# kabkabm/defensegan

Hardware: NVIDIA H100
Metric: reconstructed images/sec at R=10,L=200 (higher is better)
Workload: dtype f16

## Files before the change

### defensegan_b200/csrc/dgan_api.cu

```cuda
#include <algorithm>
#include <cmath>
#include <cstdio>
#include <cstring>
#include <memory>
#include <new>

#include "common.cuh"
#include "kernels_simt.cuh"
#include "kernels_tc.cuh"
#include "kernels_tc2.cuh"
#include "kernels_vjp.cuh"

namespace dgan {

static thread_local std::string g_last_error;
void set_error(const std::string& msg) { g_last_error = msg; }

PairTable deconv_fwd_pairs(int h_in, int w_in, int h_used, int w_used, int in_raster) {
  if (in_raster <= 0) in_raster = w_in;
  PairTable t;
  t.off.push_back(0);
  for (int i = 0; i < h_used; ++i)
    for (int j = 0; j < w_used; ++j) {
      for (int ka = 0; ka < 5; ++ka) {
// ... 1311 lines not shown
  return h->kind_names[kind].c_str();
}

int dgan_profile_read(dgan_handle h, int max_kinds, double* ms_out, int64_t* launches_out, double* flops_per_launch_out) {
  if (h == nullptr || ms_out == nullptr || launches_out == nullptr || flops_per_launch_out == nullptr) return DGAN_ERR_INVALID_ARG;
  const int nk = std::min(max_kinds, (int)h->kind_names.size());
  for (int k = 0; k < nk; ++k) {
    ms_out[k] = 0.0; launches_out[k] = 0;
    flops_per_launch_out[k] = 2.0 * h->kind_macs_per_row[k] * (double)h->n_rows_cur;
  }
  for (auto& r : h->prof) {
    DGAN_CUDA_CHECK(cudaEventSynchronize(r.b));
    float ms = 0.f;
    DGAN_CUDA_CHECK(cudaEventElapsedTime(&ms, r.a, r.b));
    if (r.kind >= 0 && r.kind < nk) { ms_out[r.kind] += ms; launches_out[r.kind]++; }
    cudaEventDestroy(r.a); cudaEventDestroy(r.b);
  }
  h->prof.clear();
  return DGAN_OK;
}

static int check_plans_impl(const dgan_desc* d, int n_rows, int n_pairs, int mutate, TcPass pass) {
  using namespace dgan;
  if (d == nullptr || n_rows <= 0 || n_pairs <= 0) { set_error("invalid argument"); return DGAN_ERR_INVALID_ARG; }
  const int n_pad = ((n_rows + 2 * kRowTile - 1) / (2 * kRowTile)) * 2 * kRowTile, n_mpairs = n_pad / (2 * kRowTile);
  Widths wd;
  if (int rc = padded_widths(d, &wd)) return rc;
  const std::string wide_target = pass == TC_PASS_TANGENT ? "Generator.3.jvp" : pass == TC_PASS_WEIGHTED ? "last.fwd.w" : "Generator.3.fwd";
  for (const TcDir& dr : tc_directions(d, pass)) {
    if (int rc = tc_dir_supported(dr)) return rc;
    Tc2Plan plan;
    int rc = tc2_plan(dr.N, dr.K, dr.tab, dr.h_grid, dr.w_grid, dr.max_acc, 0, dr.epi, dr.out_bytes, n_mpairs, n_pairs, &plan);
    if (rc) { set_error(dr.name + ": " + dgan_last_error()); return rc; }
    const bool narrow = mutate >= 12 && dr.name == "last.bwd", wide = mutate != 0 && mutate < 12 && dr.name == wide_target;
    if ((narrow || wide) && plan.stream_m.size() > 40) {
      auto mma = [&](size_t i, auto f) { TcMmaRec m = TcMmaRec::decode(plan.stream_m[i]); f(m); plan.stream_m[i] = m.encode(); };
      auto producer = [&](size_t i, auto f) { TcProducerRec p = TcProducerRec::decode(plan.stream_p[i]); f(p); plan.stream_p[i] = p.encode(); };
      auto every_mma = [&](auto f) { for (size_t i = 0; i < plan.stream_m.size(); ++i) mma(i, f); };
      switch (mutate) {
        case 1: mma(20, [](TcMmaRec& m) {
                  TcOp op = TcOp::decode(m.ops[0]);
                  op.first ^= 1u;
                  m.ops[0] = op.encode();
                });
                break;
        case 2: mma(20, [](TcMmaRec& m) {
                  for (uint32_t j = 1; j < m.maxb; ++j)
                    if (m.ops[j] != m.ops[0]) { std::swap(m.ops[0], m.ops[j]); break; }
                });
                break;
        case 3: producer(20, [](TcProducerRec& p) { p.tile[0] ^= 1u; }); break;
        case 4: producer(20, [](TcProducerRec& p) { p.pix[0] ^= 1u; }); break;
        case 5: producer(20, [](TcProducerRec& p) { p.kc ^= 1u; }); break;
        case 6: plan.eitems[0] = -1; break;
        case 7: for (size_t i = 0; i < plan.stream_p.size(); ++i)
                  producer(i, [](TcProducerRec& p) { p.dep = TC2_NSLOT; });
                break;
        case 8: producer(20, [](TcProducerRec& p) { p.off = 0xBF; }); break;
        case 9: std::swap(plan.stream_m[20], plan.stream_m[21]);
                std::swap(plan.stream_p[20], plan.stream_p[21]);
                break;
        case 10: plan.maxb = 3;
                 every_mma([](TcMmaRec& m) { m.maxb = 3; });
                 break;
        case 11: every_mma([](TcMmaRec& m) { m.maxb = 2; }); break;
        case 12: every_mma([&](TcMmaRec& m) { m.ksub = plan.ksub == 1 ? 2 : 1; }); break;
        case 13: producer(20, [](TcProducerRec& p) { p.kc |= 1u; }); break;
        default: break;
      }
    }
    std::string err;
    if ((rc = tc2_check_plan(dr.N, dr.K, dr.tab, n_mpairs, dr.epi, dr.out_bytes, plan, &err))) { set_error(dr.name + ": " + err); return rc; }
    if (mutate != 0) continue;
    for (const Tc2Kind& k : kTc2Kinds) {
      if (k.n != dr.N || k.ksub != plan.ksub || k.epi != dr.epi || k.out_bytes != dr.out_bytes || k.maxb == plan.maxb) continue;
      Tc2Plan forced;
      if ((rc = tc2_plan(dr.N, dr.K, dr.tab, dr.h_grid, dr.w_grid, dr.max_acc, k.maxb, dr.epi, dr.out_bytes, n_mpairs, n_pairs, &forced))) {
        set_error(dr.name + " (" + std::to_string(k.maxb) + " slots): " + dgan_last_error());
        return rc;
      }
      if ((rc = tc2_check_plan(dr.N, dr.K, dr.tab, n_mpairs, dr.epi, dr.out_bytes, forced, &err))) {
        set_error(dr.name + " (" + std::to_string(k.maxb) + " slots): " + err);
        return rc;
      }
    }
  }
  return 0;
}

int dgan_debug_check_plans(const dgan_desc* d, int n_rows, int n_pairs, int mutate) {
  return check_plans_impl(d, n_rows, n_pairs, mutate, TC_PASS_PROJ);
}

int dgan_debug_check_tangent_plans(const dgan_desc* d, int n_rows, int n_pairs, int mutate) {
  return check_plans_impl(d, n_rows, n_pairs, mutate, TC_PASS_TANGENT);
}

int dgan_debug_check_weighted_plans(const dgan_desc* d, int n_rows, int n_pairs, int mutate) {
  return check_plans_impl(d, n_rows, n_pairs, mutate, TC_PASS_WEIGHTED);
}
// ... 62 lines not shown
    const bool forced = (int)di == force_dir;
    const int rc = tc2_plan(dr.N, dr.K, dr.tab, dr.h_grid, dr.w_grid, dr.max_acc, forced ? force_maxb : 0, dr.epi, dr.out_bytes,
                            n_mpairs, n_pairs, &plan, forced ? force_shape : nullptr);
    if (rc) return -1;
    char line[320];
    const double mb = (double)plan.n_bytes / 1e6;
    total += mb;
    snprintf(line, sizeof line, "%s | %d | %d | %dx%d, %dx%d | %zu | %d | %lld | %lld | %.1f | %.3f | %.1f | %d | %.1f | %.1f | %lld | %s/f%d\n",
             dr.name.c_str(), dr.N, dr.K, plan.shape[0], plan.shape[1], plan.shape[2], plan.shape[3],
             plan.hdrs.size() * (size_t)n_mpairs, plan.n_slots, plan.n_steps, plan.n_mma, mb, plan.load_max / std::max(plan.load_mean, 1.0),
             100.0 * (double)plan.n_pad / (double)std::max(plan.n_mma, 1LL), plan.maxb, plan.op_ns_max / 1e3,
             plan.load_max / 1e3, plan.n_mma * plan.ksub, epi_name(dr.epi), 8 * dr.out_bytes);
    out += line;
  }
  char line[64];
  snprintf(line, sizeof line, "total staged MB per L-step | %.1f\n", total);
  out += line;
  const int n = (int)std::min(out.size(), (size_t)buf_len - 1);
  memcpy(buf, out.data(), (size_t)n);
  buf[n] = 0;
  return n;
}

int dgan_debug_plan_stats_slots(const dgan_desc* d, int n_rows, int n_pairs, int force_dir, int force_maxb, char* buf, int buf_len) {
  return plan_stats_impl(d, n_rows, n_pairs, force_dir, force_maxb, nullptr, buf, buf_len);
}

int dgan_debug_plan_stats_window(const dgan_desc* d, int n_rows, int n_pairs, int force_dir, int force_maxb, int wh, int ww,
                                 int sy, int sx, char* buf, int buf_len) {
  const int shape[4] = {wh, ww, sy, sx};
  return plan_stats_impl(d, n_rows, n_pairs, force_dir, force_maxb, shape, buf, buf_len);
}

int dgan_debug_padded_widths(const dgan_desc* d, int* out) {
  using namespace dgan;
  if (d == nullptr || out == nullptr) { set_error("invalid argument"); return DGAN_ERR_INVALID_ARG; }
  Widths w;
  if (int rc = padded_widths(d, &w)) return rc;
  out[0] = w.latent; out[1] = w.c4; out[2] = w.c2; out[3] = w.c1;
  return 0;
}

static int workspace_layout_impl(dgan_handle h, int n_rows, char* buf, int buf_len, bool weighted) {
  if (h == nullptr || n_rows <= 0 || buf == nullptr || buf_len <= 0) { set_error("invalid argument"); return -1; }
  std::string out;
  carve(h, n_rows, nullptr, &out, weighted);
  if (out.size() + 1 > (size_t)buf_len) { set_error("buffer too small"); return -1; }
  memcpy(buf, out.c_str(), out.size() + 1);
  return (int)out.size();
}

int dgan_debug_workspace_layout(dgan_handle h, int n_rows, char* buf, int buf_len) {
  return workspace_layout_impl(h, n_rows, buf, buf_len, false);
}

int dgan_debug_workspace_layout_weighted(dgan_handle h, int n_rows, char* buf, int buf_len) {
  return workspace_layout_impl(h, n_rows, buf, buf_len, true);
}

int dgan_debug_plan_stats(const dgan_desc* d, int n_rows, int n_pairs, char* buf, int buf_len) {
  return dgan_debug_plan_stats_slots(d, n_rows, n_pairs, -1, 0, buf, buf_len);
}

}
```

### defensegan_b200/csrc/kernels_tc2.cuh

```cuda
#pragma once
#include "kernels_tc.cuh"
#include "tc_records.cuh"

namespace dgan {

constexpr int TC2_SMEM_MAX = 232448;
constexpr int TC2_TILE_BYTES = 128 * 128;
constexpr int TC2_BUF_COLS = 256;
constexpr int TC2_CONSUMERS = 256;
constexpr int TC2_THREADS = TC2_CONSUMERS + 128;
constexpr int TC2_PRODUCER_REGS = 40, TC2_CONSUMER_REGS = 232;
constexpr int TC2_STORE_ROWS = 16;

constexpr int TC2_MAX_PAIRS = 80;
struct Tc2Heads {
  uint32_t off[TC2_MAX_PAIRS + 1];
};

struct __align__(16) TcItem2 {
  uint16_t q[16];
  uint32_t n_acc;
};
static_assert(sizeof(TcItem2) == 48 && offsetof(TcItem2, n_acc) == 32, "the kernel's item loads");

__host__ __device__ constexpr int tc2_acc_stride(int n_tile) { return n_tile <= 32 ? 32 : (n_tile < 64 ? 64 : n_tile); }

__host__ __device__ constexpr bool tc2_tma_epilogue(int n_tile, int epi, int out_bytes) {
  return out_bytes == 2 && n_tile >= 64 && epi != EPI_FINAL_SIGMOID1 && epi != EPI_FINAL_TANH3 && epi != EPI_FINAL_SIGMOID1_W &&
         epi != EPI_FINAL_TANH3_W;
}

constexpr int TC2_REC_BATCH = 16;
constexpr int TC2_STAGING_BYTES = TC2_REC_BATCH * (int)sizeof(TcRec);
constexpr int TC2_MREC_BYTES = TC2_NSLOT * (int)sizeof(TcRec);

__host__ __device__ constexpr int tc2_epi_tiles(int n_tile, int epi, int out_bytes) {
  return tc2_tma_epilogue(n_tile, epi, out_bytes) ? 2 : 0;
}
__host__ __device__ constexpr int tc2_ksub(int K) { return K % 64 == 0 ? 4 : K / 16; }
__host__ __device__ constexpr int tc2_a_bytes(int ksub) { return 128 * 32 * ksub; }
__host__ __device__ constexpr int tc2_b_bytes(int n_tile, int ksub) { return n_tile * 32 * ksub; }
__host__ __device__ constexpr int tc2_zero_bytes(int n_tile, int maxb, int ksub) { return maxb > 1 ? tc2_b_bytes(n_tile, ksub) : 0; }
__host__ __device__ constexpr int tc2_ring_bytes(int n_tile, int maxb, int ksub, int epi, int out_bytes) {
  const int epi_b = tc2_epi_tiles(n_tile, epi, out_bytes) * TC2_TILE_BYTES;
  const int raw = ((TC2_SMEM_MAX - 1024 - 256 - TC2_MREC_BYTES - TC2_STAGING_BYTES - epi_b - tc2_zero_bytes(n_tile, maxb, ksub)) / 1024) * 1024;
  return raw > TC2_RING_MAX_KB * 1024 ? TC2_RING_MAX_KB * 1024 : raw;
}

template <int N_TILE, int MAXB_, int KSUB_ = 4, int EPI = EPI_NONE, int OUT_BYTES = 2>
struct Tc2Cfg {
  static_assert(MAXB_ >= 1 && MAXB_ <= TC2_BUF_COLS / tc2_acc_stride(N_TILE), "more accumulator slots than columns");
  static_assert(KSUB_ >= 1 && KSUB_ <= 4, "k16 MMAs per op");
  static constexpr int KSUB = KSUB_;
  static constexpr int A_BYTES = tc2_a_bytes(KSUB);
  static constexpr int B_TILE = tc2_b_bytes(N_TILE, KSUB);
  static constexpr int A_SUB = 128 * 32, B_SUB = N_TILE * 32;
  static constexpr int MAXB = MAXB_;
  static constexpr int ACC_REGS = MAXB * N_TILE / 2;
  static constexpr bool TMA_EPI = tc2_tma_epilogue(N_TILE, EPI, OUT_BYTES);
  static constexpr int EPI_TILES = tc2_epi_tiles(N_TILE, EPI, OUT_BYTES);
  static constexpr int EPI_BYTES = EPI_TILES * TC2_TILE_BYTES;
  static constexpr int ZERO_BYTES = tc2_zero_bytes(N_TILE, MAXB, KSUB);
  static constexpr int RING_BYTES = tc2_ring_bytes(N_TILE, MAXB, KSUB, EPI, OUT_BYTES);
  static constexpr int SMEM_BYTES = RING_BYTES + ZERO_BYTES + EPI_BYTES + TC2_STAGING_BYTES + 1024 + 256 + TC2_MREC_BYTES;
};

#define TC2_KINDS(X)                                                                                                   \
  X(256, 1, 4, EPI_BIAS_RELU, __half) X(256, 1, 4, EPI_BIAS, __half) X(256, 1, 4, EPI_MASK, __half)                    \
  X(256, 1, 4, EPI_NONE, __half) X(256, 1, 4, EPI_NONE, float) X(256, 1, 4, EPI_BIAS, float)                           \
  X(128, 2, 4, EPI_BIAS_RELU, __half) X(128, 2, 4, EPI_BIAS, __half) X(128, 2, 4, EPI_MASK, __half)                    \
  X(128, 2, 4, EPI_NONE, __half) X(128, 2, 4, EPI_NONE, float) X(128, 2, 4, EPI_BIAS, float)                           \
  X(128, 1, 4, EPI_NONE, float)                                                                                        \
  X(64, 4, 4, EPI_BIAS_RELU, __half) X(64, 4, 4, EPI_BIAS, __half) X(64, 4, 4, EPI_MASK, __half)                      \
  X(64, 4, 4, EPI_NONE, __half) X(64, 4, 4, EPI_NONE, float) X(64, 4, 4, EPI_BIAS, float)                              \
// ... 62 lines not shown
__device__ __forceinline__ uint2 ld_shared_v2(uint32_t addr) {
  uint2 v;
  asm volatile("ld.shared.v2.b32 {%0, %1}, [%2];" : "=r"(v.x), "=r"(v.y) : "r"(addr));
  return v;
}
__device__ __forceinline__ uint4 ld_shared_v4(uint32_t addr) {
  uint4 v;
  asm volatile("ld.shared.v4.b32 {%0, %1, %2, %3}, [%4];" : "=r"(v.x), "=r"(v.y), "=r"(v.z), "=r"(v.w) : "r"(addr));
  return v;
}
__device__ __forceinline__ uint4 ld_shared_v4_ordered(uint32_t addr) {
  uint4 v;
  asm volatile("ld.shared.v4.b32 {%0, %1, %2, %3}, [%4];" : "=r"(v.x), "=r"(v.y), "=r"(v.z), "=r"(v.w) : "r"(addr) : "memory");
  return v;
}
__device__ __forceinline__ void bulk_load(uint32_t dst, const void* src, uint32_t bytes, uint32_t bar) {
  asm volatile("cp.async.bulk.shared::cluster.global.mbarrier::complete_tx::bytes [%0], [%1], %2, [%3];"
               ::"r"(dst), "l"(src), "r"(bytes), "r"(bar) : "memory");
}
__device__ __forceinline__ void wgmma_wait1() { asm volatile("wgmma.wait_group.sync.aligned 1;" ::: "memory"); }
template <int R> __device__ __forceinline__ void setmaxnreg_inc() { asm volatile("setmaxnreg.inc.sync.aligned.u32 %0;" ::"n"(R)); }
template <int R> __device__ __forceinline__ void setmaxnreg_dec() { asm volatile("setmaxnreg.dec.sync.aligned.u32 %0;" ::"n"(R)); }
__device__ __forceinline__ bool elect_one() {
  uint32_t pred;
  asm volatile("{\n\t.reg .pred P1;\n\telect.sync _|P1, 0xffffffff;\n\tselp.u32 %0, 1, 0, P1;\n\t}" : "=r"(pred));
  return pred != 0;
}
}

__device__ __forceinline__ int tc2_item_at(const int* __restrict__ order, int k, int pair, int n_pairs, int n_slots) {
  return k < n_slots ? __ldg(order + (size_t)k * n_pairs + pair) : -1;
}

template <int NT, int MAXB, int KSUB, int NREG>
__device__ __forceinline__ void tc2_mma_round(float (&acc)[NREG], const uint32_t (&q)[6], uint64_t da0, uint64_t db0, uint32_t zoff) {
  constexpr uint32_t DA_K = KSUB == 4 ? 2u : (uint32_t)(128 * 32 >> 4), DB_K = KSUB == 4 ? 2u : (uint32_t)(NT * 32 >> 4);
#pragma unroll
  for (int a = 0; a < MAXB; ++a) {
    const uint32_t e = TcMmaRec::Ops::get(q[a / TcMmaRec::Ops::PER_WORD], a);
    const uint32_t bs = TcOp::Slot::get(e);
    const uint64_t da = da0 + (uint64_t)(TcOp::A::get(e) * (uint32_t)(tc2_a_bytes(KSUB) >> 4));
    const uint64_t db = db0 + (uint64_t)(bs == (uint32_t)TC2_ZERO_SLOT ? zoff : bs * (uint32_t)(tc2_b_bytes(NT, KSUB) >> 4));
    const uint32_t keep = TcOp::First::get(e) ^ 1u;
#pragma unroll
    for (int k = 0; k < KSUB; ++k) ptx::Wgmma<NT>::mma(acc + a * (NT / 2), da + DA_K * k, db + DB_K * k, k > 0 ? 1u : keep);
  }
}

template <int MAXB>
__device__ __forceinline__ void tc2_pop_round(uint32_t (&q)[6]) {
  using Ops = TcMmaRec::Ops;
  static_assert(Ops::WORDS == 6, "the op queue holds every op word");
  if constexpr (MAXB >= Ops::PER_WORD) {
#pragma unroll
    for (int i = 0; i < 6; ++i) q[i] = (i + MAXB / Ops::PER_WORD < 6) ? q[i + MAXB / Ops::PER_WORD] : 0u;
  } else {
#pragma unroll
    for (int i = 0; i < 5; ++i) q[i] = __funnelshift_r(q[i], q[i + 1], Ops::BITS * MAXB);
    q[5] >>= Ops::BITS * MAXB;
  }
}

#ifdef DGAN_PROBE
constexpr int TC2_PROBE_WORDS = 16;
__device__ unsigned long long g_tc2_probe[48][160][TC2_PROBE_WORDS];
__device__ __forceinline__ unsigned long long probe_gtime() {
  unsigned long long t;
  asm volatile("mov.u64 %0, %%globaltimer;" : "=l"(t));
  return t;
}
__device__ __forceinline__ long long probe_clock_after(uint32_t w0) {
  long long t;
  asm volatile("{\n\t.reg .pred p;\n\tsetp.ge.s32 p, %1, 0;\n\tmov.u64 %0, 0;\n\t@p mov.u64 %0, %%clock64;\n\t}" : "=l"(t) : "r"(w0) : "memory");
  return t;
}
__host__ __device__ constexpr int tc2_probe_key(int n_tile, int epi, int out_bytes) {
  return (n_tile == 256 ? 0 : n_tile == 128 ? 1 : n_tile == 64 ? 2 : n_tile == 48 ? 3 : 4) * 8 + (out_bytes == 4 ? 6 : (epi < 4 ? epi : epi - 4));
}
// ... 18 lines not shown
  extern __shared__ uint8_t smem_raw[];
#ifdef DGAN_PROBE
  const long long probe_t_start = clock64();
  const unsigned long long probe_g_start = probe_gtime();
  long long probe_wait_full = 0, probe_issue = 0, probe_wait1 = 0, probe_wait0 = 0, probe_epi = 0;
  unsigned probe_rec = 0, probe_head = 0, probe_steps = 0;
#endif
  const uint32_t smem_base = (ptx::smem_u32(smem_raw) + 1023u) & ~1023u;
  const uint32_t zero_base = smem_base + Cfg::RING_BYTES;
  const uint32_t epi_base = zero_base + Cfg::ZERO_BYTES;
  const uint32_t stg_base = epi_base + Cfg::EPI_BYTES;
  const uint32_t bar_base = stg_base + TC2_STAGING_BYTES;
  const uint32_t bar_full = bar_base, bar_empty = bar_base + 64, mrec_base = bar_base + 256;

  const int warp = threadIdx.x >> 5, lane = threadIdx.x & 31;
  const uint32_t rank = ptx::cluster_ctarank();
  const int pair = blockIdx.x >> 1, n_pairs = gridDim.x >> 1;
  const uint32_t rbeg = heads.off[pair], rend = heads.off[pair + 1];

  uint4 mine = make_uint4(0, 0, 0, 0);
  if (warp == PRODUCER) {
    if (2 * rbeg + lane < 2 * rend) mine = __ldg(reinterpret_cast<const uint4*>(stream_p + rbeg) + lane);
    if (lane == 0) {
      ptx::prefetch_tmap(&tm_a);
      ptx::prefetch_tmap(&tm_b);
      if (TMA_EPI) ptx::prefetch_tmap(&tm_out);
      for (int s = 0; s < TC2_NSLOT; ++s) {
        ptx::mbar_init(bar_full + 8 * s, 1);
        ptx::mbar_init(bar_empty + 8 * s, 2 * TC2_CONSUMERS / 32);
      }
      ptx::fence_barrier_init();
    }
  }
  if constexpr (Cfg::ZERO_BYTES > 0) {
    if (threadIdx.x < TC2_CONSUMERS) {
      for (uint32_t i = threadIdx.x; i < (uint32_t)Cfg::ZERO_BYTES / 16u; i += TC2_CONSUMERS) ptx::st_shared_v4(zero_base + 16u * i, 0u, 0u, 0u, 0u);
      ptx::fence_proxy_async_smem();
    }
  }
  ptx::cluster_sync();
#ifdef DGAN_PROBE
  const long long probe_t_entry = clock64();
#endif
  pdl_launch_dependents();
  pdl_wait();
#ifdef DGAN_PROBE
  const long long probe_t_go = clock64();
  unsigned probe_h0 = (unsigned)probe_t_go;
  bool probe_new_item = true;
#endif

  if (warp >= PRODUCER) {
    ptx::setmaxnreg_dec<TC2_PRODUCER_REGS>();
    if (warp == PRODUCER) {
      const TcRec* __restrict__ stream = stream_p;
      uint32_t it = 0;
      const uint32_t ring = stg_base;
      for (uint32_t base = rbeg; base < rend; base += TC2_REC_BATCH) {
        ptx::st_shared_v4(ring + lane * 16u, mine.x, mine.y, mine.z, mine.w);
        __syncwarp();
        if (2 * (base + TC2_REC_BATCH) + lane < 2 * rend) mine = __ldg(reinterpret_cast<const uint4*>(stream + base + TC2_REC_BATCH) + lane);
        const uint32_t cnt = min((uint32_t)TC2_REC_BATCH, rend - base);
        for (uint32_t i = 0; i < cnt; ++i, ++it) {
          const uint4 r0 = ptx::ld_shared_v4(ring + i * 32u);
          const uint2 r1 = ptx::ld_shared_v2(ring + i * 32u + 16u);
          const uint32_t slot = it & (TC2_NSLOT - 1);
          using P = TcProducerRec;
// ... 60 lines not shown
#ifdef DGAN_PROBE
        const long long probe_w0 = clock64();
        if (probe_new_item) probe_head += (unsigned)probe_w0 - probe_h0;
        probe_new_item = false;
#endif
        ptx::mbar_wait(bar_full + 8 * slot, phase);
#ifdef DGAN_PROBE
        const long long probe_w1 = clock64();
        probe_wait_full += probe_w1 - probe_w0;
        if (it == 0 && threadIdx.x == 0) g_tc2_probe[tc2_probe_key(N_TILE, EPI, (int)sizeof(TOUT))][blockIdx.x][7] = probe_gtime();
#endif
        const uint4 r0 = ptx::ld_shared_v4_ordered(mrec_base + slot * (uint32_t)sizeof(TcRec));
        const uint4 r1 = ptx::ld_shared_v4_ordered(mrec_base + slot * (uint32_t)sizeof(TcRec) + 16u);
        flags = TcMmaRec::Flags::get(r0.x);
#ifdef DGAN_PROBE
        const unsigned probe_rec_step = (unsigned)probe_clock_after(r0.x) - (unsigned)probe_w1;
        probe_rec += probe_rec_step;
#endif
        const int nA = TcMmaRec::NA::get(r0.x), n_rounds = TcMmaRec::Rounds::get(r0.x);
        const uint32_t sa = smem_base + (TcMmaRec::Off::get(r0.x) << 10);
        const uint64_t da0 = KSUB == 4 ? make_smem_desc_sw128(sa + (uint32_t)wg * 64u * 128u) : make_smem_desc_sw32(sa + (uint32_t)wg * 64u * 32u);
        const uint32_t sb = sa + (uint32_t)nA * A_BYTES;
        const uint64_t db0 = KSUB == 4 ? make_smem_desc_sw128(sb) : make_smem_desc_sw32(sb);
        const uint32_t zoff = (zero_base - sb) >> 4;
        uint32_t q[6] = {r0.z, r0.w, r1.x, r1.y, r1.z, r1.w};
#ifdef DGAN_PROBE
        long long probe_step_wait = 0;
#endif
        ptx::fence_operands(acc);
        ptx::wgmma_fence();
        for (int r = 0; r < n_rounds; ++r) {
          tc2_mma_round<N_TILE, Cfg::MAXB, KSUB>(acc, q, da0, db0, zoff);
          tc2_pop_round<Cfg::MAXB>(q);
          ptx::wgmma_commit();
#ifdef DGAN_PROBE
          const long long probe_c0 = clock64();
#endif
          ptx::wgmma_wait1();
#ifdef DGAN_PROBE
          probe_step_wait += clock64() - probe_c0;
#endif
          if (r == 0) {
            __syncwarp();
            if (!(flags & TcMmaRec::FIRST) && lane < 2) ptx::mbar_arrive_cluster(bar_empty + 8 * ((it - 1) & (TC2_NSLOT - 1)), (uint32_t)lane);
          }
        }
        ptx::fence_operands(acc);
#ifdef DGAN_PROBE
        probe_wait1 += probe_step_wait;
        probe_issue += clock64() - probe_w1 - probe_step_wait - probe_rec_step;
#endif
        ++ri; ++it;
      } while (!(flags & TcMmaRec::LAST));
#ifdef DGAN_PROBE
      const long long probe_d0 = clock64();
#endif
      ptx::wgmma_wait0();
      ptx::fence_operands(acc);
#ifdef DGAN_PROBE
      const long long probe_e0 = clock64();
      probe_wait0 += probe_e0 - probe_d0;
#endif
      __syncwarp();
      if (lane < 2) ptx::mbar_arrive_cluster(bar_empty + 8 * ((it - 1) & (TC2_NSLOT - 1)), (uint32_t)lane);

      const int mp = tc2_item_mp(item_e);
      auto q_of = [&](int a) { return (int)__shfl_sync(0xffffffffu, q_mine, a); };
// ... 237 lines not shown
};
static uint32_t tc2_box_k(int K) { return tc2_ksub(K) == 4 ? 64u : 16u; }
struct TcDir {
  std::string name, kind;
  int N = 0, K = 0, P_in = 0, P_out = 0, n_tiles = 0;
  PairTable tab;
  int h_grid = 0, w_grid = 0;
  int max_acc = 1;
  int epi = EPI_NONE, out_bytes = 2, bias_pstride = 0;
  int ld = 0, col0 = 0, out_ld = 0;
  int n_real = 0;
  std::string base_kind;
  __half* w = nullptr;
  CUtensorMap tm_b{};
  int force_maxb = 0;
  std::vector<std::pair<int, Tc2Schedule>> by_mpairs;
};

static int tc2_maxb(int N) { return TC2_BUF_COLS / tc2_acc_stride(N); }

struct Tc2HostStep {
  int kc = 0, nA = 0, nB = 0, n_rounds = 0;
  int a_pix[TC2_MAX_A] = {0, 0, 0, 0};
  uint8_t b_ent[TC2_MAX_BSLOTS] = {0};
  uint8_t ops[TC2_OP_BYTES] = {0};
  int n_real = 0;
  int bytes = 0;
};
struct Tc2HostItem {
  TcItem2 hdr{};
  std::vector<Tc2HostStep> steps;
  double stage_bytes = 0.0;
  long long n_ops = 0;
};

static void tc2_build_item(const PairTable& tab, const std::vector<int>& qs, int N, int K, int max_b, int max_a,
                           int step_max_bytes, Tc2HostItem* out) {
  const int ksub = tc2_ksub(K), kch = K / (16 * ksub), a_bytes = tc2_a_bytes(ksub), b_tile = tc2_b_bytes(N, ksub);
  out->hdr = TcItem2{};
  out->hdr.n_acc = (uint32_t)qs.size();
  for (size_t a = 0; a < qs.size(); ++a) out->hdr.q[a] = (uint16_t)qs[a];
  out->steps.clear();
  std::vector<std::pair<int, std::vector<std::pair<int, int>>>> by_p;
  for (size_t a = 0; a < qs.size(); ++a)
    for (int e = tab.off[qs[a]]; e < tab.off[qs[a] + 1]; ++e) {
      const int p = tab.pairs[e].x, t = tab.pairs[e].y;
      size_t g = 0;
      for (; g < by_p.size(); ++g)
        if (by_p[g].first == p) break;
      if (g == by_p.size()) by_p.push_back({p, {}});
      by_p[g].second.push_back({t, (int)a});
    }
  std::sort(by_p.begin(), by_p.end(), [](const auto& l, const auto& r) { return l.first < r.first; });
  for (auto& g : by_p)
    std::stable_sort(g.second.begin(), g.second.end(), [](const auto& l, const auto& r) { return l.second < r.second; });
  std::vector<std::pair<int, std::vector<std::pair<int, int>>>> px;
  const int ent_cap = std::min(TC2_MAX_BSLOTS, std::max(1, (step_max_bytes - a_bytes) / b_tile));
  for (auto& g : by_p)
    for (size_t b0 = 0; b0 < g.second.size(); b0 += (size_t)ent_cap)
      px.push_back({g.first, std::vector<std::pair<int, int>>(g.second.begin() + b0,
                                                               g.second.begin() + std::min(g.second.size(), b0 + (size_t)ent_cap))});
  const int max_rounds = TC2_OP_BYTES / max_b;
  struct Group { size_t i0, i1; };
  std::vector<Group> groups;
  {
    size_t i0 = 0;
// ... 35 lines not shown
    st.nA = (int)(G.i1 - G.i0);
    std::fill(st.ops, st.ops + TC2_OP_BYTES, TC2_PAD_OP);
    int slot_of[32], cnt[8] = {0, 0, 0, 0, 0, 0, 0, 0};
    for (int t = 0; t < 32; ++t) slot_of[t] = -1;
    for (size_t i = G.i0; i < G.i1; ++i) {
      st.a_pix[i - G.i0] = px[i].first;
      for (auto& ta : px[i].second) {
        const int t = ta.first, acc = ta.second;
        if (slot_of[t] < 0) {
          slot_of[t] = st.nB;
          st.b_ent[st.nB++] = (uint8_t)t;
        }
        const bool first = !(seen & (1u << acc));
        const int r = cnt[acc]++;
        st.ops[r * max_b + acc] = TcOp{(uint32_t)(i - G.i0), (uint32_t)slot_of[t], first ? 1u : 0u}.encode();
        st.n_rounds = std::max(st.n_rounds, r + 1);
        st.n_real += 1;
        seen |= 1u << acc;
      }
    }
    st.bytes = st.nA * a_bytes + st.nB * b_tile;
    out->steps.push_back(st);
  }
  const size_t n_groups = out->steps.size();
  for (int kc = 1; kc < kch; ++kc)
    for (size_t gi = 0; gi < n_groups; ++gi) {
      Tc2HostStep sk = out->steps[gi];
      sk.kc = kc;
      for (int o = 0; o < TC2_OP_BYTES; ++o) sk.ops[o] = (uint8_t)TcOp::First::put(sk.ops[o], 0u);
      out->steps.push_back(sk);
    }
  out->stage_bytes = 0.0;
  out->n_ops = 0;
  for (auto& stp : out->steps) { out->stage_bytes += stp.bytes; out->n_ops += (long long)stp.n_rounds * max_b; }
}

static void tc2_enumerate_windows(int h_grid, int w_grid, int wh, int ww, int sy, int sx, std::vector<std::vector<int>>* wins) {
  wins->clear();
  for (int by = 0; by < h_grid; by += wh * sy)
    for (int bx = 0; bx < w_grid; bx += ww * sx)
      for (int ry = 0; ry < sy; ++ry)
        for (int rx = 0; rx < sx; ++rx) {
          std::vector<int> qs;
          for (int i = 0; i < wh; ++i)
            for (int j = 0; j < ww; ++j) {
              const int y = by + ry + i * sy, x = bx + rx + j * sx;
              if (y < h_grid && x < w_grid) qs.push_back(y * w_grid + x);
            }
          if (!qs.empty()) wins->push_back(qs);
        }
}

#ifndef DGAN_STEP_MAX_KB
#define DGAN_STEP_MAX_KB 48
#endif
#ifndef DGAN_STEP_MAX_KB_N64
#define DGAN_STEP_MAX_KB_N64 64
#endif
#ifndef DGAN_COST_EPI_KB
#define DGAN_COST_EPI_KB 24.0
#endif
#ifndef DGAN_COST_FIXED_KB
#define DGAN_COST_FIXED_KB 48.0
#endif
#ifndef DGAN_COST_NS_PER_KB
#define DGAN_COST_NS_PER_KB 6.8
#endif
#ifndef DGAN_COST_OP_NS
#define DGAN_COST_OP_NS 103.0
#endif
#ifndef DGAN_COST_STEP_NS
#define DGAN_COST_STEP_NS 942.0
#endif
#ifndef DGAN_COST_OP_MIN_N
#define DGAN_COST_OP_MIN_N 32
#endif
#ifndef TC2_REFINE_BUDGET
#define TC2_REFINE_BUDGET (1LL << 26)
#endif

struct Tc2Plan {
  int shape[4] = {1, 1, 1, 1};
  int n_slots = 0, n_pairs = 0;
  std::vector<TcItem2> hdrs;
  std::vector<TcRec> stream_p, stream_m;
  std::vector<uint32_t> stream_off;
  std::vector<int> eitems;
  long long n_mma = 0, n_pad = 0, n_steps = 0, n_bytes = 0;
  double load_max = 0.0, load_mean = 0.0;
  double op_ns_max = 0.0;
  int maxb = 1, ring_bytes = 0;
  int ksub = 4;
};

static double tc2_op_ns(int N, int ksub) {
  return DGAN_COST_OP_NS * (double)std::max(N, DGAN_COST_OP_MIN_N) / 64.0 * (double)ksub / 4.0;
}

static int tc2_search(int N, int K, const PairTable& tab, int h_grid, int w_grid, int max_acc, int force_maxb, int epi,
                      int out_bytes, int n_mpairs, int n_pairs, const int* force_shape, Tc2Plan* plan,
                      std::vector<Tc2HostItem>* best_items, std::vector<std::vector<int>>* best_lists) {
  const int max_a = TC2_MAX_A;
  const int step_kb = (N == 64 && K == 128) ? DGAN_STEP_MAX_KB_N64 : DGAN_STEP_MAX_KB;
  const int ksub = tc2_ksub(K);
  const double op_ns = tc2_op_ns(N, ksub);
  double best_cost = 1e300;
  plan->maxb = 0;
  std::vector<std::vector<int>> wins;
  for (const Tc2Kind& kind : kTc2Kinds) {
    if (kind.n != N || kind.ksub != ksub || kind.epi != epi || kind.out_bytes != out_bytes) continue;
    if (force_maxb > 0 && kind.maxb != force_maxb) continue;
    const int mb = kind.maxb, ring = tc2_ring_bytes(N, mb, ksub, epi, out_bytes);
    const int step_max = std::min((ring / 3) & ~1023, step_kb * 1024);
    for (int wh = 1; wh <= 2; ++wh)
      for (int ww = 1; ww <= 8; ++ww)
        for (int sy = 1; sy <= (wh > 1 ? 2 : 1); ++sy)
          for (int sx = 1; sx <= (ww > 1 ? 2 : 1); ++sx) {
            if (wh * ww > std::min(max_acc, mb) || wh > h_grid || ww > std::max(w_grid, 1)) continue;
            if (force_shape != nullptr && (wh != force_shape[0] || ww != force_shape[1] || sy != force_shape[2] || sx != force_shape[3])) continue;
            tc2_enumerate_windows(h_grid, std::max(w_grid, 1), wh, ww, sy, sx, &wins);
            std::vector<Tc2HostItem> items(wins.size());
            for (size_t i = 0; i < wins.size(); ++i) tc2_build_item(tab, wins[i], N, K, mb, max_a, step_max, &items[i]);
            std::vector<double> icost(items.size());
// ... 29 lines not shown
                  if (peak < best_peak - 1e-9) { best_peak = peak; bq = Q; bi = (int)i; bj = -1; }
                  for (size_t j = 0; j < lists[Q].size(); ++j) {
                    const double cj = cost_of(lists[Q][j]);
                    if (cj >= ci) continue;
                    peak = std::max(load[P] - ci + cj, load[Q] + ci - cj);
                    if (peak < best_peak - 1e-9) { best_peak = peak; bq = Q; bi = (int)i; bj = (int)j; }
                  }
                }
              }
              if (bi < 0) break;
              const int it_i = lists[P][(size_t)bi];
              const double ci = cost_of(it_i);
              if (bj < 0) {
                lists[P].erase(lists[P].begin() + bi);
                lists[bq].push_back(it_i);
                load[P] -= ci; load[bq] += ci;
              } else {
                const int it_j = lists[bq][(size_t)bj];
                const double cj = cost_of(it_j);
                lists[P][(size_t)bi] = it_j; lists[bq][(size_t)bj] = it_i;
                load[P] += cj - ci; load[bq] += ci - cj;
              }
            }
            for (auto& l : lists)
              std::stable_sort(l.begin(), l.end(), [&](int a, int b) { return cost_of(a) > cost_of(b); });
            const double makespan = *std::max_element(load.begin(), load.end());
            if (makespan < best_cost) {
              best_cost = makespan;
              plan->load_max = makespan;
              plan->load_mean = std::accumulate(load.begin(), load.end(), 0.0) / (double)n_pairs;
              plan->shape[0] = wh; plan->shape[1] = ww; plan->shape[2] = sy; plan->shape[3] = sx;
              plan->maxb = mb; plan->ring_bytes = ring;
              plan->op_ns_max = 0.0;
              for (size_t pr = 0; pr < lists.size(); ++pr)
                if (load[pr] == makespan) {
                  for (int idx : lists[pr]) plan->op_ns_max += op_ns * (double)items[(size_t)(idx / n_mpairs)].n_ops;
                  break;
                }
              best_items->swap(items); best_lists->swap(lists);
            }
          }
  }
  if (plan->maxb == 0) { set_error("no tensor-core kernel instantiation for this layer-direction"); return DGAN_ERR_UNSUPPORTED; }
  plan->ksub = ksub;
  return 0;
}

static int tc2_encode_streams(int N, int n_mpairs, int n_pairs, const std::vector<Tc2HostItem>& items,
                              const std::vector<std::vector<int>>& lists, Tc2Plan* plan) {
  const int max_b = plan->maxb, ring_bytes = plan->ring_bytes, ksub = plan->ksub;
  plan->n_pairs = n_pairs;
  size_t n_slots = 0;
  for (auto& l : lists) n_slots = std::max(n_slots, l.size());
  plan->n_slots = (int)n_slots;
  std::vector<int>& eitems = plan->eitems;
  eitems.assign(n_slots * (size_t)n_pairs, -1);
  std::vector<uint32_t>& stream_off = plan->stream_off;
  stream_off.assign((size_t)n_pairs + 1, 0);
  std::vector<TcRec>& stream_p = plan->stream_p;
  std::vector<TcRec>& stream_m = plan->stream_m;
  stream_p.clear(); stream_m.clear();
  long long n_mma = 0, n_pad = 0, n_steps = 0, n_bytes = 0;
  for (size_t pr = 0; pr < lists.size(); ++pr) {
    stream_off[pr] = (uint32_t)stream_m.size();
    std::vector<std::pair<int, int>> region;
    int cursor = 0;
    for (size_t k = 0; k < lists[pr].size(); ++k) {
      const int win = lists[pr][k] / n_mpairs, mp = lists[pr][k] % n_mpairs;
      if ((uint32_t)win > TcItemWindow::mask || (uint32_t)mp > TcItemMp::mask) { set_error("tensor-core schedule limits exceeded"); return DGAN_ERR_UNSUPPORTED; }
      eitems[k * (size_t)n_pairs + pr] = tc2_item_word(win, mp);
      const Tc2HostItem& itm = items[(size_t)win];
      for (size_t j = 0; j < itm.steps.size(); ++j) {
        const Tc2HostStep& hs = itm.steps[j];
        const int kb = (hs.bytes + 1023) / 1024;
        if (kb * 1024 > ring_bytes) { set_error("tensor-core step larger than the operand ring"); return DGAN_ERR_UNSUPPORTED; }
        if (cursor + kb > ring_bytes / 1024) cursor = 0;
        const int beg = cursor, end = cursor + kb;
        cursor = end;
        int dep = TC2_NSLOT;
        const int kidx = (int)region.size();
        for (int d = 1; d <= TC2_NSLOT && d <= kidx; ++d) {
          const auto& rg = region[(size_t)(kidx - d)];
          if (rg.first < end && beg < rg.second) { dep = d; break; }
        }
        if (dep == 1 && j > 0) { set_error("tensor-core step overlaps the step before it (ring too small)"); return DGAN_ERR_UNSUPPORTED; }
        region.push_back({beg, end});
        TcMmaRec m;
        m.off = (uint32_t)beg; m.nA = (uint32_t)hs.nA; m.n_rounds = (uint32_t)hs.n_rounds; m.maxb = (uint32_t)max_b; m.ksub = (uint32_t)ksub;
        m.flags = (j == 0 ? TcMmaRec::FIRST : 0u) | (j + 1 == itm.steps.size() ? TcMmaRec::LAST : 0u);
        std::copy(hs.ops, hs.ops + hs.n_rounds * max_b, m.ops);
        stream_m.push_back(m.encode());
        TcProducerRec p;
        p.off = (uint32_t)beg; p.kc = (uint32_t)hs.kc; p.nA = (uint32_t)hs.nA; p.nB = (uint32_t)hs.nB; p.dep = (uint32_t)dep; p.mp = (uint32_t)mp;
        std::copy(hs.a_pix, hs.a_pix + TC2_MAX_A, p.pix);
        std::copy(hs.b_ent, hs.b_ent + TC2_MAX_BSLOTS, p.tile);
        stream_p.push_back(p.encode());
        n_mma += hs.n_rounds * max_b; n_pad += hs.n_rounds * max_b - hs.n_real;
        n_steps += 1; n_bytes += 2LL * hs.nA * tc2_a_bytes(ksub) + (long long)hs.nB * tc2_b_bytes(N, ksub);
      }
    }
  }
  stream_off[(size_t)n_pairs] = (uint32_t)stream_m.size();
  plan->hdrs.resize(items.size());
  for (size_t i = 0; i < items.size(); ++i) plan->hdrs[i] = items[i].hdr;
  plan->n_mma = n_mma; plan->n_pad = n_pad; plan->n_steps = n_steps; plan->n_bytes = n_bytes;
  return 0;
}

static int tc2_plan(int N, int K, const PairTable& tab, int h_grid, int w_grid, int max_acc, int force_maxb, int epi,
                    int out_bytes, int n_mpairs, int n_pairs, Tc2Plan* plan, const int* force_shape = nullptr) {
  std::vector<Tc2HostItem> items;
  std::vector<std::vector<int>> lists;
  const int rc = tc2_search(N, K, tab, h_grid, w_grid, max_acc, force_maxb, epi, out_bytes, n_mpairs, n_pairs, force_shape,
                            plan, &items, &lists);
  return rc ? rc : tc2_encode_streams(N, n_mpairs, n_pairs, items, lists, plan);
}

static int tc2_check_plan(int N, int K, const PairTable& tab, int n_mpairs, int epi, int out_bytes, const Tc2Plan& pl,
                          std::string* err) {
  auto fail = [&](const std::string& m) { *err = m; return DGAN_ERR_INVALID_ARG; };
  const int ksub = tc2_ksub(K), kch = K / (16 * ksub), a_bytes = tc2_a_bytes(ksub), b_tile = tc2_b_bytes(N, ksub);
  const int max_acc = pl.maxb;
  if (pl.ksub != ksub) return fail("plan's k16 MMAs per op disagree with the direction's channels");
  if (!tc2_has_kind(N, max_acc, ksub, epi, out_bytes)) return fail("no kernel instantiation with these accumulator slots per round");
  const int ring_bytes = tc2_ring_bytes(N, max_acc, ksub, epi, out_bytes);
  const size_t n_pairs = (size_t)pl.n_pairs;
  if (pl.stream_off.size() != n_pairs + 1) return fail("stream_off size");
  if (pl.stream_p.size() != pl.stream_m.size()) return fail("stream sizes differ");
  if (pl.eitems.size() != (size_t)pl.n_slots * n_pairs) return fail("eitems size");
  std::vector<int> assigned(pl.hdrs.size() * (size_t)n_mpairs, 0);
  for (const TcItem2& h : pl.hdrs) {
    if (h.n_acc < 1 || (int)h.n_acc > max_acc) return fail("window with too many accumulators");
    for (uint32_t a = 0; a < h.n_acc; ++a)
      if ((size_t)h.q[a] + 1 >= tab.off.size()) return fail("window pixel out of range");
  }
  struct Step { int beg, end; };
  for (size_t pr = 0; pr < n_pairs; ++pr) {
    const uint32_t r_beg = pl.stream_off[pr], r_end = pl.stream_off[pr + 1];
// ... 8 lines not shown
      const TcMmaRec m = TcMmaRec::decode(pl.stream_m[ri]);
      const TcProducerRec p0 = TcProducerRec::decode(pl.stream_p[ri]);
      const int k = (int)steps.size();
      const int nA = (int)p0.nA, nB = (int)p0.nB, dep = (int)p0.dep, kc = (int)p0.kc;
      Step st{(int)p0.off, 0};
      if (m.off != p0.off || m.nA != p0.nA) return fail("MMA record disagrees with the producer record");
      if (nA < 1 || nA > TC2_MAX_A || nB > TC2_MAX_BSLOTS || kc >= kch) return fail("step field out of range");
      st.end = st.beg + (nA * a_bytes + nB * b_tile + 1023) / 1024;
      if (st.end * 1024 > ring_bytes) return fail("step region outside the ring");
      if (dep < 1 || dep > TC2_NSLOT) return fail("dep out of range");
      const uint32_t flags = m.flags;
      const int n_rounds = (int)m.n_rounds;
      if ((int)m.maxb != max_acc) return fail("MMA record disagrees with the plan on the accumulator slots per round");
      if ((int)m.ksub != ksub) return fail("MMA record disagrees with the instantiation on the k16 sub-tiles per op");
      if (n_rounds < 1 || n_rounds * max_acc > TC2_OP_BYTES) return fail("round count out of range");
      if (dep == 1 && !(flags & TcMmaRec::FIRST)) return fail("ring deadlock: a step waits for the step before it, which is released only after it");
      if (flags & TcMmaRec::FIRST) {
        if (in_item) return fail("item starts inside an item");
        in_item = true; ++item_k;
        if (item_k >= pl.n_slots) return fail("more items than slots");
        const int e = pl.eitems[(size_t)item_k * n_pairs + pr];
        if (e < 0) return fail("stream has an item the epilogue list lacks");
        win = tc2_item_window(e); mp = tc2_item_mp(e);
        if ((size_t)win >= pl.hdrs.size() || mp >= n_mpairs) return fail("item index out of range");
        if (assigned[(size_t)win * n_mpairs + mp]++) return fail("item assigned twice");
        seen = 0;
        last_kp.assign(pl.hdrs[win].n_acc, {-1, -1});
        contrib.assign(pl.hdrs[win].n_acc, {});
      }
      if (!in_item) return fail("step outside an item");
      if ((int)p0.mp != mp) return fail("row pair of a step differs from its item");
      const TcItem2& hdr = pl.hdrs[win];
      for (int oi = 0; oi < n_rounds * max_acc; ++oi) {
        const TcOp op = TcOp::decode(m.ops[oi]);
        const int a_idx = (int)op.a, slot = (int)op.slot, acc = oi % max_acc;
        const bool first = op.first != 0;
        if (m.ops[oi] & ~TcOp::USED) return fail("op field out of range");
        if (slot == TC2_ZERO_SLOT) {
          if (max_acc == 1) return fail("zero-tile op in an instantiation without a zero tile");
          if (first) return fail("zero-tile op overwrites its accumulator");
          continue;
        }
        if (a_idx >= nA) return fail("op reads an A tile the step does not stage");
        if (acc >= (int)hdr.n_acc) return fail("op writes past the window's accumulators");
        if (slot >= nB) return fail("op reads a B slot the step does not stage");
        if (p0.tile[slot] > TcProducerRec::Tile::mask) return fail("weight tile entry out of range");
        const int p = (int)p0.pix[a_idx];
        const bool unseen = !(seen & (1u << acc));
        if (first != unseen) return fail(first ? "overwrite of a live accumulator" : "accumulate into an uninitialised accumulator");
        const std::pair<int, int> kp{kc, p};
        if (!(last_kp[acc] < kp)) return fail("accumulation order is not canonical (k-chunk major, pixel ascending)");
        last_kp[acc] = kp;
        contrib[acc].push_back({p * 32 + (int)p0.tile[slot], kc});
        seen |= 1u << acc;
      }
      for (int c = k - 1; c >= 0 && c >= k - 4 * TC2_NSLOT; --c) {
        const Step& o = steps[(size_t)c];
        if (!(o.beg < st.end && st.beg < o.end)) continue;
        if (c > k - dep) return fail("ring hazard: a region may be overwritten while it can still be read");
      }
      steps.push_back(st);
      if (flags & TcMmaRec::LAST) {
        for (uint32_t a = 0; a < hdr.n_acc; ++a) {
          std::vector<std::pair<int, int>> want;
          for (int kc = 0; kc < kch; ++kc)
            for (int e2 = tab.off[hdr.q[a]]; e2 < tab.off[hdr.q[a] + 1]; ++e2) want.push_back({tab.pairs[e2].x * 32 + tab.pairs[e2].y, kc});
          std::vector<std::pair<int, int>> got = contrib[a];
          std::sort(want.begin(), want.end()); std::sort(got.begin(), got.end());
          if (want != got) return fail("an item's MMAs do not cover exactly its pair list");
        }
        in_item = false;
      }
// ... 74 lines not shown
```

Measured before the change: 2578.

## Skip zero-tile wgmma ops via per-round mask-specialized MMA variants

For instantiations with 2-4 accumulator slots and full k-chunks, each round now builds a bitmask of its non-padding ops and dispatches to a template variant that issues wgmma only for real ops. Padding ops that multiplied by the zeroed B tile are no longer sent to the tensor cores, and the zero tile is no longer initialized in those configurations. The commit moves into the op helper, the plan checker rejects rounds that contain no real op, and new statistics and test mutations are added. The switch over mask variants adds code size and some branching per round.

```diff
diff --git a/defensegan_b200/csrc/dgan_api.cu b/defensegan_b200/csrc/dgan_api.cu
--- a/defensegan_b200/csrc/dgan_api.cu
+++ b/defensegan_b200/csrc/dgan_api.cu
@@ -1367,7 +1367,8 @@
     Tc2Plan plan;
     int rc = tc2_plan(dr.N, dr.K, dr.tab, dr.h_grid, dr.w_grid, dr.max_acc, 0, dr.epi, dr.out_bytes, n_mpairs, n_pairs, &plan);
     if (rc) { set_error(dr.name + ": " + dgan_last_error()); return rc; }
-    const bool narrow = mutate >= 12 && dr.name == "last.bwd", wide = mutate != 0 && mutate < 12 && dr.name == wide_target;
+    const bool narrow = (mutate == 12 || mutate == 13) && dr.name == "last.bwd";
+    const bool wide = mutate != 0 && mutate != 12 && mutate != 13 && dr.name == wide_target;
     if ((narrow || wide) && plan.stream_m.size() > 40) {
       auto mma = [&](size_t i, auto f) { TcMmaRec m = TcMmaRec::decode(plan.stream_m[i]); f(m); plan.stream_m[i] = m.encode(); };
       auto producer = [&](size_t i, auto f) { TcProducerRec p = TcProducerRec::decode(plan.stream_p[i]); f(p); plan.stream_p[i] = p.encode(); };
@@ -1401,6 +1402,22 @@
         case 11: every_mma([](TcMmaRec& m) { m.maxb = 2; }); break;
         case 12: every_mma([&](TcMmaRec& m) { m.ksub = plan.ksub == 1 ? 2 : 1; }); break;
         case 13: producer(20, [](TcProducerRec& p) { p.kc |= 1u; }); break;
+        case 14: mma(20, [](TcMmaRec& m) {
+                   for (uint32_t j = 0; j < m.maxb; ++j) m.ops[j] = TC2_PAD_OP;
+                 });
+                 break;
+        case 15: {
+                   bool done = false;
+                   for (size_t i = 20; i < plan.stream_m.size() && !done; ++i)
+                     mma(i, [&](TcMmaRec& m) {
+                       for (uint32_t j = 0; j < m.n_rounds * m.maxb && !done; ++j)
+                         if (TcOp::decode(m.ops[j]).slot == (uint32_t)TC2_ZERO_SLOT) {
+                           m.ops[j] = (uint8_t)TcOp::First::put(m.ops[j], 1u);
+                           done = true;
+                         }
+                     });
+                   break;
+                 }
         default: break;
       }
     }
@@ -1529,6 +1546,27 @@
   return plan_stats_impl(d, n_rows, n_pairs, force_dir, force_maxb, shape, buf, buf_len);
 }
 
+int dgan_debug_plan_issue_stats(const dgan_desc* d, int n_rows, int n_pairs, char* buf, int buf_len) {
+  using namespace dgan;
+  if (d == nullptr || n_rows <= 0 || n_pairs <= 0 || buf == nullptr || buf_len <= 0) { set_error("invalid argument"); return -1; }
+  const int n_pad = ((n_rows + 2 * kRowTile - 1) / (2 * kRowTile)) * 2 * kRowTile, n_mpairs = n_pad / (2 * kRowTile);
+  Widths wd;
+  if (padded_widths(d, &wd) != 0) return -1;
+  std::string out = "direction | slots | k16 MMAs issued | zero-tile k16 MMAs skipped | busiest pair: est. tensor us, issued\n";
+  for (const TcDir& dr : tc_directions(d)) {
+    Tc2Plan plan;
+    if (tc2_plan(dr.N, dr.K, dr.tab, dr.h_grid, dr.w_grid, dr.max_acc, 0, dr.epi, dr.out_bytes, n_mpairs, n_pairs, &plan)) return -1;
+    char line[200];
+    snprintf(line, sizeof line, "%s | %d | %lld | %lld | %.1f\n", dr.name.c_str(), plan.maxb, plan.n_issued * plan.ksub,
+             (plan.n_mma - plan.n_issued) * plan.ksub, plan.op_ns_issued_max / 1e3);
+    out += line;
+  }
+  const int n = (int)std::min(out.size(), (size_t)buf_len - 1);
+  memcpy(buf, out.data(), (size_t)n);
+  buf[n] = 0;
+  return n;
+}
+
 int dgan_debug_padded_widths(const dgan_desc* d, int* out) {
   using namespace dgan;
   if (d == nullptr || out == nullptr) { set_error("invalid argument"); return DGAN_ERR_INVALID_ARG; }
diff --git a/defensegan_b200/csrc/kernels_tc2.cuh b/defensegan_b200/csrc/kernels_tc2.cuh
--- a/defensegan_b200/csrc/kernels_tc2.cuh
+++ b/defensegan_b200/csrc/kernels_tc2.cuh
@@ -40,6 +40,7 @@
 __host__ __device__ constexpr int tc2_ksub(int K) { return K % 64 == 0 ? 4 : K / 16; }
 __host__ __device__ constexpr int tc2_a_bytes(int ksub) { return 128 * 32 * ksub; }
 __host__ __device__ constexpr int tc2_b_bytes(int n_tile, int ksub) { return n_tile * 32 * ksub; }
+__host__ __device__ constexpr bool tc2_issues_zero_ops(int maxb, int ksub) { return maxb > 4 || (maxb > 1 && ksub < 4); }
 __host__ __device__ constexpr int tc2_zero_bytes(int n_tile, int maxb, int ksub) { return maxb > 1 ? tc2_b_bytes(n_tile, ksub) : 0; }
 __host__ __device__ constexpr int tc2_ring_bytes(int n_tile, int maxb, int ksub, int epi, int out_bytes) {
   const int epi_b = tc2_epi_tiles(n_tile, epi, out_bytes) * TC2_TILE_BYTES;
@@ -168,18 +169,45 @@
   return k < n_slots ? __ldg(order + (size_t)k * n_pairs + pair) : -1;
 }
 
-template <int NT, int MAXB, int KSUB, int NREG>
-__device__ __forceinline__ void tc2_mma_round(float (&acc)[NREG], const uint32_t (&q)[6], uint64_t da0, uint64_t db0, uint32_t zoff) {
+template <int NT, int MAXB, int KSUB, uint32_t MASK, int NREG>
+__device__ __forceinline__ void tc2_mma_ops(float (&acc)[NREG], const uint32_t (&q)[6], uint64_t da0, uint64_t db0, uint32_t zoff) {
   constexpr uint32_t DA_K = KSUB == 4 ? 2u : (uint32_t)(128 * 32 >> 4), DB_K = KSUB == 4 ? 2u : (uint32_t)(NT * 32 >> 4);
 #pragma unroll
   for (int a = 0; a < MAXB; ++a) {
+    if (!((MASK >> a) & 1u)) continue;
     const uint32_t e = TcMmaRec::Ops::get(q[a / TcMmaRec::Ops::PER_WORD], a);
     const uint32_t bs = TcOp::Slot::get(e);
     const uint64_t da = da0 + (uint64_t)(TcOp::A::get(e) * (uint32_t)(tc2_a_bytes(KSUB) >> 4));
-    const uint64_t db = db0 + (uint64_t)(bs == (uint32_t)TC2_ZERO_SLOT ? zoff : bs * (uint32_t)(tc2_b_bytes(NT, KSUB) >> 4));
+    const uint32_t boff = bs * (uint32_t)(tc2_b_bytes(NT, KSUB) >> 4);
+    const uint64_t db = db0 + (uint64_t)(tc2_issues_zero_ops(MAXB, KSUB) && bs == (uint32_t)TC2_ZERO_SLOT ? zoff : boff);
     const uint32_t keep = TcOp::First::get(e) ^ 1u;
 #pragma unroll
     for (int k = 0; k < KSUB; ++k) ptx::Wgmma<NT>::mma(acc + a * (NT / 2), da + DA_K * k, db + DB_K * k, k > 0 ? 1u : keep);
+  }
+  ptx::wgmma_commit();
+}
+
+template <int NT, int MAXB, int KSUB, int NREG>
+__device__ __forceinline__ void tc2_mma_round(float (&acc)[NREG], const uint32_t (&q)[6], uint64_t da0, uint64_t db0, uint32_t zoff) {
+  if constexpr (tc2_issues_zero_ops(MAXB, KSUB) || MAXB == 1) {
+    tc2_mma_ops<NT, MAXB, KSUB, (1u << MAXB) - 1u>(acc, q, da0, db0, zoff);
+  } else {
+    static_assert(MAXB <= TcMmaRec::Ops::PER_WORD, "a round's op bytes share the queue's first word");
+    uint32_t set = 0;
+#pragma unroll
+    for (int a = 0; a < MAXB; ++a)
+      set |= (TcOp::Slot::get(TcMmaRec::Ops::get(q[0], a)) != (uint32_t)TC2_ZERO_SLOT ? 1u : 0u) << a;
+    switch (set) {
+#define TC2_ROUND_VARIANT(M) \
+  case M:                    \
+    if constexpr (M < (1u << MAXB)) tc2_mma_ops<NT, MAXB, KSUB, M>(acc, q, da0, db0, zoff); \
+    break;
+      TC2_ROUND_VARIANT(1u) TC2_ROUND_VARIANT(2u) TC2_ROUND_VARIANT(3u) TC2_ROUND_VARIANT(4u) TC2_ROUND_VARIANT(5u)
+      TC2_ROUND_VARIANT(6u) TC2_ROUND_VARIANT(7u) TC2_ROUND_VARIANT(8u) TC2_ROUND_VARIANT(9u) TC2_ROUND_VARIANT(10u)
+      TC2_ROUND_VARIANT(11u) TC2_ROUND_VARIANT(12u) TC2_ROUND_VARIANT(13u) TC2_ROUND_VARIANT(14u) TC2_ROUND_VARIANT(15u)
+#undef TC2_ROUND_VARIANT
+      default: __builtin_unreachable();
+    }
   }
 }
 
@@ -264,7 +292,7 @@
       ptx::fence_barrier_init();
     }
   }
-  if constexpr (Cfg::ZERO_BYTES > 0) {
+  if constexpr (Cfg::ZERO_BYTES > 0 && tc2_issues_zero_ops(MAXB, KSUB)) {
     if (threadIdx.x < TC2_CONSUMERS) {
       for (uint32_t i = threadIdx.x; i < (uint32_t)Cfg::ZERO_BYTES / 16u; i += TC2_CONSUMERS) ptx::st_shared_v4(zero_base + 16u * i, 0u, 0u, 0u, 0u);
       ptx::fence_proxy_async_smem();
@@ -391,7 +419,6 @@
         for (int r = 0; r < n_rounds; ++r) {
           tc2_mma_round<N_TILE, Cfg::MAXB, KSUB>(acc, q, da0, db0, zoff);
           tc2_pop_round<Cfg::MAXB>(q);
-          ptx::wgmma_commit();
 #ifdef DGAN_PROBE
           const long long probe_c0 = clock64();
 #endif
@@ -695,6 +722,7 @@
   std::vector<Tc2HostStep> steps;
   double stage_bytes = 0.0;
   long long n_ops = 0;
+  long long n_issued = 0;
 };
 
 static void tc2_build_item(const PairTable& tab, const std::vector<int>& qs, int N, int K, int max_b, int max_a,
@@ -796,7 +824,12 @@
     }
   out->stage_bytes = 0.0;
   out->n_ops = 0;
-  for (auto& stp : out->steps) { out->stage_bytes += stp.bytes; out->n_ops += (long long)stp.n_rounds * max_b; }
+  out->n_issued = 0;
+  for (auto& stp : out->steps) {
+    out->stage_bytes += stp.bytes;
+    out->n_ops += (long long)stp.n_rounds * max_b;
+    out->n_issued += tc2_issues_zero_ops(max_b, ksub) ? (long long)stp.n_rounds * max_b : (long long)stp.n_real;
+  }
 }
 
 static void tc2_enumerate_windows(int h_grid, int w_grid, int wh, int ww, int sy, int sx, std::vector<std::vector<int>>* wins) {
@@ -850,9 +883,10 @@
   std::vector<TcRec> stream_p, stream_m;
   std::vector<uint32_t> stream_off;
   std::vector<int> eitems;
-  long long n_mma = 0, n_pad = 0, n_steps = 0, n_bytes = 0;
+  long long n_mma = 0, n_pad = 0, n_issued = 0, n_steps = 0, n_bytes = 0;
   double load_max = 0.0, load_mean = 0.0;
   double op_ns_max = 0.0;
+  double op_ns_issued_max = 0.0;
   int maxb = 1, ring_bytes = 0;
   int ksub = 4;
 };
@@ -948,9 +982,13 @@
               plan->shape[0] = wh; plan->shape[1] = ww; plan->shape[2] = sy; plan->shape[3] = sx;
               plan->maxb = mb; plan->ring_bytes = ring;
               plan->op_ns_max = 0.0;
+              plan->op_ns_issued_max = 0.0;
               for (size_t pr = 0; pr < lists.size(); ++pr)
                 if (load[pr] == makespan) {
-                  for (int idx : lists[pr]) plan->op_ns_max += op_ns * (double)items[(size_t)(idx / n_mpairs)].n_ops;
+                  for (int idx : lists[pr]) {
+                    plan->op_ns_max += op_ns * (double)items[(size_t)(idx / n_mpairs)].n_ops;
+                    plan->op_ns_issued_max += op_ns * (double)items[(size_t)(idx / n_mpairs)].n_issued;
+                  }
                   break;
                 }
               best_items->swap(items); best_lists->swap(lists);
@@ -976,7 +1014,7 @@
   std::vector<TcRec>& stream_p = plan->stream_p;
   std::vector<TcRec>& stream_m = plan->stream_m;
   stream_p.clear(); stream_m.clear();
-  long long n_mma = 0, n_pad = 0, n_steps = 0, n_bytes = 0;
+  long long n_mma = 0, n_pad = 0, n_issued = 0, n_steps = 0, n_bytes = 0;
   for (size_t pr = 0; pr < lists.size(); ++pr) {
     stream_off[pr] = (uint32_t)stream_m.size();
     std::vector<std::pair<int, int>> region;
@@ -1012,6 +1050,7 @@
         std::copy(hs.b_ent, hs.b_ent + TC2_MAX_BSLOTS, p.tile);
         stream_p.push_back(p.encode());
         n_mma += hs.n_rounds * max_b; n_pad += hs.n_rounds * max_b - hs.n_real;
+        n_issued += tc2_issues_zero_ops(max_b, ksub) ? hs.n_rounds * max_b : hs.n_real;
         n_steps += 1; n_bytes += 2LL * hs.nA * tc2_a_bytes(ksub) + (long long)hs.nB * tc2_b_bytes(N, ksub);
       }
     }
@@ -1019,7 +1058,7 @@
   stream_off[(size_t)n_pairs] = (uint32_t)stream_m.size();
   plan->hdrs.resize(items.size());
   for (size_t i = 0; i < items.size(); ++i) plan->hdrs[i] = items[i].hdr;
-  plan->n_mma = n_mma; plan->n_pad = n_pad; plan->n_steps = n_steps; plan->n_bytes = n_bytes;
+  plan->n_mma = n_mma; plan->n_pad = n_pad; plan->n_issued = n_issued; plan->n_steps = n_steps; plan->n_bytes = n_bytes;
   return 0;
 }
 
@@ -1094,12 +1133,16 @@
       if ((int)p0.mp != mp) return fail("row pair of a step differs from its item");
       const TcItem2& hdr = pl.hdrs[win];
       for (int oi = 0; oi < n_rounds * max_acc; ++oi) {
+        if (oi % max_acc == 0) {
+          int real = 0;
+          for (int a = 0; a < max_acc; ++a) real += TcOp::decode(m.ops[oi + a]).slot != (uint32_t)TC2_ZERO_SLOT;
+          if (real == 0) return fail("round without a real op (it would commit an empty wgmma group)");
+        }
         const TcOp op = TcOp::decode(m.ops[oi]);
         const int a_idx = (int)op.a, slot = (int)op.slot, acc = oi % max_acc;
         const bool first = op.first != 0;
         if (m.ops[oi] & ~TcOp::USED) return fail("op field out of range");
         if (slot == TC2_ZERO_SLOT) {
-          if (max_acc == 1) return fail("zero-tile op in an instantiation without a zero tile");
           if (first) return fail("zero-tile op overwrites its accumulator");
           continue;
         }
```

Result: faster. 2694 (median of 6 runs) (+4.5%).
